# Yujia-Yan/Transkun

Hardware: AMD Instinct MI355X
Metric: semi-CRF logProb+backward steps/sec at T=1024, NBatch=352 (higher is better)
Workload: dtype f32; 1 GPU; NeuralSemiCRFInterval(score, noise).logProb(intervals) fwd+bwd through the public API (Python interval lists packed inside the timed region), T=1024, NBatch=352 per GPU, fp32, exact-hash randn-like scores resident in HBM; T=1024, NBatch=352, impl=0, parallelism=chains sharded, 1 rank(s) seen by the process group, no data-path collective

## Files before the change

include/semicrf_hip.h:

```cpp
#ifndef SEMICRF_HIP_H
#define SEMICRF_HIP_H

#include <stddef.h>
#include <stdint.h>

#ifdef __cplusplus
extern "C" {
#endif

#define SEMICRF_ABI_VERSION 2

#define SEMICRF_OK 0
#define SEMICRF_EINVAL 1
#define SEMICRF_EWORKSPACE 2
#define SEMICRF_ELAUNCH 3
#define SEMICRF_ETIMEOUT 4

#define SEMICRF_OP_LOGZ_FWD 0
#define SEMICRF_OP_LOGZ_BWD 1
#define SEMICRF_OP_VITERBI 2
#define SEMICRF_OP_EVAL_PATH 3
#define SEMICRF_OP_INTERVAL_SCORE 4
#define SEMICRF_OP_SAMPLE 5
#define SEMICRF_OP_VITERBI_NBEST 6
// ... 13 lines not shown

#define SEMICRF_SCORE_BF16X3 4
#define SEMICRF_LEN_BF16X3 16

typedef void* semicrf_stream_t;

int semicrf_abi_version(void);
const char* semicrf_last_error(void);
size_t semicrf_workspace_bytes(int op, int T, int B);

int semicrf_workspace_register(void* ws, size_t ws_bytes);
int semicrf_workspace_unregister(void* ws);

void semicrf_set_impl(int impl);
int semicrf_get_impl(void);

int semicrf_debug_device_status(void);

int semicrf_async_error(void);

int semicrf_debug_wg_ticket(int n_spine, int grid, int block);

void semicrf_debug_score_variant(int variant);

int semicrf_logz_fwd(const float* score, const float* noise, int T, int B,
                     float* logZ, float* v, void* ws, size_t ws_bytes, semicrf_stream_t stream);

int semicrf_logz_bwd(const float* score, const float* noise, const float* v, const float* logZ,
                     const float* gout, int T, int B, float* dScore, float* dNoise, float* q_out,
                     void* ws, size_t ws_bytes, semicrf_stream_t stream);
// ... 261 lines not shown
```

transkun_amd/_lib.py:

```python
from __future__ import annotations

import collections
import ctypes
import os
from typing import Optional

import torch

_HERE = os.path.dirname(os.path.abspath(__file__))
LIB_PATH = os.environ.get("SEMICRF_LIB") or os.path.join(_HERE, "libsemicrf_hip.so")

OP_LOGZ_FWD, OP_LOGZ_BWD, OP_VITERBI, OP_EVAL_PATH, OP_INTERVAL_SCORE, OP_SAMPLE, OP_VITERBI_NBEST, OP_POSTERIORS = range(8)
OP_MARGINAL_DECODE = 8
OP_EXPECTATION = 9
OP_MBR_SELECT = 10
OP_MARGINAL_DECODE_TOL = 11
OP_ATTRIBUTE_HEADS = 12
OP_ATTRIBUTE_HEADS_BWD = 13
HEADS_ROW_TILE = 64
HEADS_SLICE = 64
HEADS_BWD_ROW_CHUNK = 512
ATTENTION_MAX_L = 256
ATTENTION_MAX_D = 64
TOL_MAX = 8
# ... 15 lines not shown
                ("step", ctypes.c_float), ("rectified", ctypes.c_int32), ("pad_", ctypes.c_int32)]


class AdaBeliefGroups(ctypes.Structure):
    _fields_ = [("n", ctypes.c_int32), ("pad_", ctypes.c_int32), ("g", AdaBeliefGroup * OPTIM_MAX_GROUPS)]


_SIGS = {
    "semicrf_abi_version": (ctypes.c_int, []),
    "semicrf_last_error": (ctypes.c_char_p, []),
    "semicrf_workspace_bytes": (_sz, [_i, _i, _i]),
    "semicrf_workspace_register": (_i, [_vp, _sz]),
    "semicrf_workspace_unregister": (_i, [_vp]),
    "semicrf_set_impl": (None, [_i]),
    "semicrf_get_impl": (ctypes.c_int, []),
    "semicrf_debug_device_status": (ctypes.c_int, []),
    "semicrf_async_error": (ctypes.c_int, []),
    "semicrf_logz_bwd_f": (_i, [_vp, _vp, _vp, _vp, _vp, _i, _i, _vp, _vp, _vp, _i, _vp, _sz, _vp]),
    "semicrf_logprob_bwd_f": (_i, [_vp, _vp, _vp, _vp, _vp, _i, _i, _i, _vp, _i64, _vp, _vp, _vp, _i, _vp, _sz, _vp]),
    "semicrf_logprob_path_table_supported": (_i, [_i, _i]),
    "semicrf_logprob_fwd_t": (_i, [_vp, _vp, _i, _i, _vp, _i64, _vp, _vp, _vp, _vp, _vp, _vp, _sz, _vp]),
    "semicrf_logprob_bwd_t": (_i, [_vp, _vp, _vp, _vp, _vp, _i, _i, _i, _vp, _i64, _vp, _vp, _vp, _i, _vp, _vp, _sz, _vp]),
    "semicrf_debug_wg_ticket": (_i, [_i, _i, _i]),
    "semicrf_debug_score_variant": (None, [_i]),
    "semicrf_logz_fwd": (_i, [_vp, _vp, _i, _i, _vp, _vp, _vp, _sz, _vp]),
    "semicrf_logz_bwd": (_i, [_vp, _vp, _vp, _vp, _vp, _i, _i, _vp, _vp, _vp, _vp, _sz, _vp]),
    "semicrf_viterbi": (_i, [_vp, _vp, _i, _i, _vp, _i, _vp, _i64, _vp, _vp, _sz, _vp]),
    "semicrf_sample": (_i, [_vp, _vp, _vp, _i, _i, _i64, _i, ctypes.c_uint64, _vp, _vp, _i64, _vp, _vp, _sz, _vp]),
    "semicrf_viterbi_nbest": (_i, [_vp, _vp, _i, _i, _i, _vp, _i, _vp, _i64, _vp, _vp, _vp, _vp, _sz, _vp]),
    "semicrf_posteriors": (_i, [_vp, _vp, _vp, _vp, _vp, _i, _i, _vp, _vp, _vp, _vp, _vp, _vp, _vp, _sz, _vp]),
# ... 190 lines not shown
    with torch.cuda.device(device):
        rc = load().semicrf_workspace_register(ctypes.c_void_p(ws.data_ptr()), ctypes.c_size_t(ws.numel()))
    if rc != 0:
        check(rc, "semicrf_workspace_register")
    _LEASES[key] = ws
    while len(_LEASES) > _LEASE_MAX:
        _, old = _LEASES.popitem(last=False)
        load().semicrf_workspace_unregister(ctypes.c_void_p(old.data_ptr()))
    return ws


def set_impl(impl: int) -> None:
    load().semicrf_set_impl(int(impl))


def device_status() -> int:
    return int(load().semicrf_debug_device_status())


def async_error() -> int:
    return int(load().semicrf_async_error())


def get_impl() -> int:
    return int(load().semicrf_get_impl())
```

transkun_amd/csrc/api.hip:

```cpp
#include <stdarg.h>
#include <string.h>
#include <stdlib.h>
#include <atomic>
#include <mutex>
#include <unordered_map>
#include "common.h"
#include "attention_math.h"

namespace semicrf {

static thread_local char g_err[512] = "";
static std::atomic<int> g_impl{0};

void set_error(const char* fmt, ...)
{
    va_list ap;
    va_start(ap, fmt);
    vsnprintf(g_err, sizeof(g_err), fmt, ap);
    va_end(ap);
}

void launch_rowseq_sweep(int mode, int dir, const float* score, const float* noise, int T, int B, float* u,
                         int* code, float* out_last, hipStream_t stream);
void launch_marginals(const float* score, const float* noise, const float* v, const float* q,
// ... 81 lines not shown
                   const float* bias, const float* w2, const float* b2, int zero_cols, int accumulate, hipStream_t stream);
size_t proj_tn_workspace_bytes(long long M, int R, int N);
size_t proj_nn3_workspace_bytes(int K, int N);
int launch_proj_nn3(const float* A, long long lda, long long M, int K, const float* B, long long ldb, int N, float* out, long long ldout,
                    const float* bias, const float* w2, const float* b2, int zero_cols, int accumulate, void* ws, size_t ws_bytes,
                    hipStream_t stream);
void launch_merge_weights_fwd(const float* W, const float* bias, int D, int size, int rows, float* Wm, float* bm, float* WmT, hipStream_t stream);
void launch_merge_weights_bwd(const float* W, const float* bias, const float* dWm, const float* dbm, int D, int size, float* dW, float* dbias,
                              float* ws, hipStream_t stream);
size_t merge_weights_bwd_workspace_bytes(int size);
void launch_stage_linear(const float* W, const float* bias, int D, int size, int rows_pad, float* BT, float* Wqd, float* w2, float* b2,
                         hipStream_t stream);
int launch_proj_tn(const float* A, long long lda, long long M, int R, int extra_col0, int total_rows, const float* X, long long ldx, int N,
                   float* dW, long long lddw, float* db, void* ws, size_t ws_bytes, hipStream_t stream);
size_t persist_workspace_bytes(int T, int B);
size_t sample_workspace_bytes(int T, int nB);
size_t posterior_workspace_bytes(int T, int B);
size_t expectation_workspace_bytes(int T, int B);
void launch_alpha_from(const float* score, const float* noise, const int* start, int T, int B, float* v, float* logZ, hipStream_t stream);
void launch_expectation(const float* score, const float* noise, const float* weight, const float* nweight, const float* v, const float* q,
                        int T, int B, float* E, float* H, void* ws, hipStream_t stream);
void launch_covariance(const float* score, const float* noise, const float* weight, const float* nweight, const float* gout, int T, int B,
                       float* C, float* Cn, const void* ws, hipStream_t stream);
void launch_posteriors(const float* score, const float* noise, const float* v, const float* q, const float* logZ, int T, int B,
                       float* node, float* begin, float* end, float* single, float* noiseP, float* entropy, void* ws,
                       hipStream_t stream);
void launch_interval_marginals(const float* score, const float* v, const float* q, const float* logZ, int T, int B, const int* pairs,
                               int K, const int* offsets, float* out, hipStream_t stream);
size_t marginal_decode_workspace_bytes(int T, int B);
void launch_marginal_decode(const float* score, const float* v, const float* q, const float* logZ, int T, int B, const float* tau,
// ... 131 lines not shown
    std::lock_guard<std::mutex> lk(g_lease_mu);
    auto it = g_leases.find(ws);
    if (it != g_leases.end()) it->second.clean = false;
}

}

using namespace semicrf;

extern "C" {

int semicrf_abi_version(void) { return SEMICRF_ABI_VERSION; }
const char* semicrf_last_error(void) { return g_err; }
void semicrf_set_impl(int impl) { g_impl.store(impl); }
int semicrf_get_impl(void) { return g_impl.load(); }
int semicrf_debug_device_status(void) { return read_and_clear_device_status(); }
int semicrf_async_error(void) { return (int)take_async_error(); }
int semicrf_debug_wg_ticket(int n_spine, int grid, int block) { return persist_wg_ticket(n_spine, grid, block); }
void semicrf_debug_score_variant(int variant) { set_score_variant(variant); }

int semicrf_workspace_register(void* ws, size_t ws_bytes)
{
    SEMICRF_CHECK_ARG(ws != nullptr && ws_bytes > 0, "workspace is NULL or empty");
    if (ensure_abort_word(nullptr)) { set_error("could not hand the abort word to the device"); return SEMICRF_ELAUNCH; }
    std::lock_guard<std::mutex> lk(g_lease_mu);
    g_leases[ws] = Lease{ws_bytes, -1, 0, 0, false, 0u};
    return SEMICRF_OK;
}

int semicrf_workspace_unregister(void* ws)
// ... 1124 lines not shown
```

transkun_amd/csrc/persist.hip:

```cpp
#include <atomic>
#include <stdlib.h>
#include "common.h"
#include "pathscore.h"

#ifndef SEMICRF_PANEL_PROBES
#define SEMICRF_PANEL_PROBES 0
#endif

#ifndef SEMICRF_PROBE_TASKS
#define SEMICRF_PROBE_TASKS 0
#endif
#ifndef SEMICRF_PROBE_HIST
#define SEMICRF_PROBE_HIST 0
#endif

#ifndef SEMICRF_CT_DBG
#define SEMICRF_CT_DBG -1
#endif

namespace semicrf {

constexpr int PB = 16;
#ifndef SEMICRF_RING
#define SEMICRF_RING 4
// ... 14 lines not shown
#endif
#ifndef SEMICRF_BANDX_WGSTRIDE
#define SEMICRF_BANDX_WGSTRIDE 3
#endif
#ifndef SEMICRF_BANDX_WAVES
#define SEMICRF_BANDX_WAVES 1
#endif
#ifndef SEMICRF_BANDX_K0
#define SEMICRF_BANDX_K0 8
#endif
constexpr int NBT = RING + NNEAR;
constexpr int FAR0 = RING + NNEAR;
constexpr int RS = 4;
constexpr int GS = RS;
constexpr int GP = 32;
#ifndef SEMICRF_TPT
#define SEMICRF_TPT 12
#endif
constexpr int TPT = SEMICRF_TPT;
#ifndef SEMICRF_LEADT
#define SEMICRF_LEADT 4
#endif
constexpr int LEADT = SEMICRF_LEADT;
__host__ __device__ inline int nfull_of(int q) { return q + 1 - LEADT >= 0 ? (q + 1 - LEADT) / TPT : 0; }
__host__ __device__ inline int nparts_of(int q) { return nfull_of(q) + 1; }
__host__ __device__ inline void part_tiles(int q, int part, int& m0, int& m1)
{
    m0 = part * TPT;
    m1 = part < nfull_of(q) ? m0 + TPT : q + 1;
}
#ifndef SEMICRF_NT
#define SEMICRF_NT 640
#endif
constexpr int NT = SEMICRF_NT;
constexpr int MAX_CHUNKS = 16;
constexpr float LOG2E = 1.4426950408889634f;
constexpr float LN2 = 0.6931471805599453f;
constexpr int SPIN_LIMIT = 1 << 20;
constexpr int SPIN_LIMIT_LDS = 1 << 24;
constexpr float RESC_LIFT = 96.0f, RESC_HI = 108.0f, RESC_EARLY = 56.0f;
constexpr unsigned CTRL_INIT = 0xffffffffu;
constexpr unsigned U_EMPTY = 0xffffffffu;

constexpr size_t CTRL_WORDS = 256;
constexpr int CTRL_EXIT = 64;
// ... 19 lines not shown
    int panelWaves;
    int hybridPanelWaves;
    int hybridStart;
    int zeroWaves;
    unsigned tag;
    int selfclean;
    unsigned expect_gen;
    unsigned dbg;
    unsigned* ctrl;
    u64* ts;
    unsigned* ug;
    unsigned* ug_other;
    int gradLazyShort;
    int bandWaves;
    u64* farg;
    float* u_out;
    float* last_out;
    int* code;
    const float* vfwd;
    const float* logZ;
    const float* gout;
    int gstride;
    float gscale;
    float* dScore;
    float* dNoise;
    const int* pathPairs;
    const int* pathOffsets;
    int pathK;
    int pathSpine;
    float* pathOut;
// ... 18 lines not shown
__device__ __forceinline__ u64 make_granule(unsigned tag, float v)
{
    return ((u64)tag << 32) | (u64)__float_as_uint(v);
}
__device__ __forceinline__ u64 make_granule_key(unsigned tag, float v, int key)
{
    return ((u64)(((tag & 0xffffu) << 16) | ((unsigned)key & 0xffffu)) << 32) | (u64)__float_as_uint(v);
}
__device__ __forceinline__ void store_granule(u64* p, u64 g)
{
    __hip_atomic_store(p, g, __ATOMIC_RELAXED, __HIP_MEMORY_SCOPE_AGENT);
}
__device__ __forceinline__ u64 load_granule(const u64* p)
{
    return __hip_atomic_load(p, __ATOMIC_RELAXED, __HIP_MEMORY_SCOPE_AGENT);
}

template <typename Tp>
__device__ __forceinline__ Tp kernarg_again(size_t off)
{
    typedef __attribute__((address_space(4))) const char ka_t;
    ka_t* ka = (ka_t*)__builtin_amdgcn_kernarg_segment_ptr();
    asm volatile("" : "+s"(ka));
    return *(__attribute__((address_space(4))) const Tp*)(ka + off);
}

template <int DIR>
__device__ __forceinline__ int frame_of(int p, int T) { return DIR == 0 ? p : T - 1 - p; }

template <int DIR>
// ... 340 lines not shown
    int* const fcons = (int*)(lds + LDS_CTL) + NRBUF + RING + NNSLOT + fw;
    float* const dScore = P.dScore;
    float gz = 0.f, lzc = 0.f;
    if (GRAD && NNEAR > 0 && cvalid) { gz = P.gout[(size_t)c * P.gstride] * P.gscale; lzc = P.logZ[c]; }
    __builtin_amdgcn_s_setprio(SEMICRF_FAR_PRIO);
    const bool fprobe = SEMICRF_PANEL_PROBES && (DBGF(P) & 16u) && cbase_is_first && lane == 0;
    const int nfar = NNEAR > 0 ? NFARW : __builtin_amdgcn_readfirstlane(P.nfarw);
    if (fw >= nfar) return;
    for (int k = RING + fw; k < K; k += nfar) {
        if (fprobe && k < 64) P.ts[640 + k] = __builtin_amdgcn_s_memrealtime();
        const int prow = k * PB + r;
        const bool rvalid = cvalid && prow < T;
        const int prow_c = prow < T ? prow : T - 1;
        float aM = SEMICRF_NEG_INF, aS = 0.f;
        int aK = 0x7fffffff;
        const int nparts = k >= FAR0 ? nparts_of(k - FAR0) : 0;
        u64 eq[4] = {0, 0, 0, 0};
        if (SEMICRF_FAR_EARLY && rvalid && nparts > 0) {
#pragma unroll
            for (int i = 0; i < 4; ++i)
                if (i < nparts) eq[i] = load_granule(farg + ((size_t)i * T + prow) * Bs + c);
        }
        float ncell[NNEAR > 0 ? NNEAR : 1][PB];
        float arow = 0.f;
        if (NNEAR > 0) {
            int spins = 0;
            while (lds_flag_load(nready + k % NNSLOT) != k + 1) {
                __builtin_amdgcn_s_sleep(1);
                if (spin_abort(ctrl, spins, SPIN_LIMIT_LDS, 11)) break;
            }
            const char* nb = lds + LDS_NEAR + (k % NNSLOT) * NEAR_SLOT_BYTES;
#pragma unroll
            for (int n = 0; n < NNEAR; ++n)
#pragma unroll
                for (int u = 0; u < PB; ++u) ncell[n][u] = *(const float*)(nb + n * TILE_BYTES + u * (PB * RS * 4) + (r * RS + ch) * 4);
            if (GRAD) arow = rvalid ? (((const float*)(nb + NNEAR * TILE_BYTES))[lane] - lzc) * LOG2E : 0.f;
// ... 50 lines not shown
                }
            }
        }
        if (fprobe && k < 64) P.ts[832 + k] = __builtin_amdgcn_s_memrealtime();
        if (rvalid && nparts > 0) {
            for (int p0 = 0; p0 < nparts; p0 += 4) {
                const int np = nparts - p0 < 4 ? nparts - p0 : 4;
                u64 gq[4];
                bool have[4] = {false, false, false, false};
                int spins = 0;
                bool first = SEMICRF_FAR_EARLY && p0 == 0;
                while (true) {
#pragma unroll
                    for (int i = 0; i < 4; ++i)
                        if (i < np && !have[i])
                            gq[i] = first ? eq[i] : load_granule(farg + ((size_t)(p0 + i) * T + prow) * Bs + c);
                    first = false;
                    bool all = true;
#pragma unroll
                    for (int i = 0; i < 4; ++i)
                        if (i < np && !have[i]) {
                            const bool ok = MODE == 0 ? (unsigned)(gq[i] >> 32) == tag : (unsigned)(gq[i] >> 48) == (tag & 0xffffu);
                            if (ok) have[i] = true;
                            else all = false;
                        }
                    if (all) break;
                    __builtin_amdgcn_s_sleep(1);
                    if (spin_abort(ctrl, spins, SPIN_LIMIT, 3)) break;
                }
#pragma unroll
                for (int i = 0; i < 4; ++i)
// ... 311 lines not shown
                    gr = load_granule(pathg + c);
                    if ((unsigned)(gr >> 32) == ptag) break;
                    __builtin_amdgcn_s_sleep(8);
                    if (spin_abort(ctrl, spins, SPIN_LIMIT, 15)) { ok = false; break; }
                }
                pathOut[c] = ok ? __uint_as_float((unsigned)gr) - mine * sc : __uint_as_float(0x7fc00000u);
            }
            if (GRAD) {
                float dv = gz * fexp2(arow + mine + draw - 2.0f * sp);
                if (pdiag) dv = dv + nadd;
                dScore[((size_t)frow * T + frow) * Bs + c] = dv;
            }
            if (MODE == 1) code[(size_t)c * T + frow] = (mykey + 1) | (sp > 0.0f ? 0x40000000 : 0);
        }
        if (SEMICRF_PANEL_PROBES && trace) ts[k] = __builtin_amdgcn_s_memrealtime();
    }
}

#ifndef SEMICRF_GRAD_AUX
#define SEMICRF_GRAD_AUX 2
#endif
constexpr int GRAD_AUX = SEMICRF_GRAD_AUX;
#ifndef SEMICRF_CELL_AUX
#define SEMICRF_CELL_AUX 2
#endif
constexpr int CELL_AUX = SEMICRF_CELL_AUX;
#ifndef SEMICRF_PNS
#define SEMICRF_PNS 3
#endif
constexpr int PNS = SEMICRF_PNS;
// ... 89 lines not shown
                 : "v"(addr), "n"(0 * XR + 0 * XH), "n"(0 * XR + 1 * XH), "n"(1 * XR + 0 * XH), "n"(1 * XR + 1 * XH),
                   "n"(2 * XR + 0 * XH), "n"(2 * XR + 1 * XH), "n"(3 * XR + 0 * XH), "n"(3 * XR + 1 * XH));
}
__device__ __forceinline__ void panel_wait_younger(int y)
{
    if (y >= 44) wait_vmcnt<44>();
    else if (y >= 36) wait_vmcnt<36>();
    else if (y >= 28) wait_vmcnt<28>();
    else if (y >= 20) wait_vmcnt<20>();
    else if (y >= 10) wait_vmcnt<10>();
    else wait_vmcnt<0>();
}

struct PanelTask { int k, part, g, q4; };

__device__ __forceinline__ void panel_tt_decode(int tt, PanelTask& t)
{
    if (tt < LEADT - 1) { t.part = 0; t.k = FAR0 + tt; return; }
    tt -= LEADT - 1;
    int a = 0;
    while (tt >= TPT * (a + 1) * (a + 2) / 2) ++a;
    tt -= TPT * a * (a + 1) / 2;
    const int q = a * TPT + tt / (a + 1) + LEADT - 1;
    t.part = tt % (a + 1);
    t.k = FAR0 + q;
}
__device__ __forceinline__ void panel_task_decode(const SweepParams& P, int task, PanelTask& t)
{
    t.q4 = task & 3;
    const int t2 = task >> 2;
    t.g = t2 % P.nPanelGroups;
    panel_tt_decode(t2 / P.nPanelGroups, t);
}

__device__ __forceinline__ bool panel_next_task(const SweepParams& P, PanelTask& t)
{
    int task = 0;
    if ((threadIdx.x & 63) == 0) task = (int)(atomicAdd(P.ctrl + 2, 1u) + 1u);
    task = __builtin_amdgcn_readfirstlane(task) + P.taskBase;
    if (task >= P.nTasks) return false;
    panel_task_decode(P, task, t);
    return true;
}

template <int MODE, int DIR, bool GRAD>
__device__ __forceinline__ void panel_role(const SweepParams& P, char* lds, int wslot, int hist_role = 0, int first_task = -1)
{
// ... 34 lines not shown
    while (true) {
        PanelTask tk;
        if (first_task >= 0 && first_task < P.nTasks) {
            panel_task_decode(P, first_task, tk);
#if SEMICRF_STAGGER > 0
            for (int i = 0, n = tk.k - FAR0 < 48 ? tk.k - FAR0 : 48; i < n; ++i) __builtin_amdgcn_s_sleep(SEMICRF_STAGGER);
#endif
        } else if (!panel_next_task(P, tk)) break;
        first_task = -1;
        if (SEMICRF_PROBE_TASKS && (dbg & 256u) && tk.k == RING && tk.part == 0 && tk.g == 0 && tk.q4 == 0) tracer = true;
        u64* const tsp = P.ts + (3 * T) / 2 + 5 * tn;
        const bool tr = SEMICRF_PROBE_TASKS && tracer && lane == 0 && 5 * tn + 5 <= T / 2;
        if (tr) tsp[0] = __builtin_amdgcn_s_memrealtime();
        const int q = tk.k - FAR0;
        int m0, m1;
        part_tiles(q, tk.part, m0, m1);
        const int k = tk.k, part = tk.part, g = tk.g, q4 = tk.q4;
        const int pbase = k * PB + q4 * 4;
        if (pbase >= T) continue;
        const int c = c0 + g * GP + q8 * 4;
        const bool cvalid = c < c1;
        const int cl = cvalid ? c : c0;

        float aM[4][4], aS[4][4];
        int aK[4][4];
#pragma unroll
        for (int rr = 0; rr < 4; ++rr)
#pragma unroll
            for (int i = 0; i < 4; ++i) { aM[rr][i] = SEMICRF_NEG_INF; aS[rr][i] = 0.f; aK[rr][i] = 0x7fffffff; }

        float arow[4][4], gz[4];
// ... 216 lines not shown
            if (tprobe) { P.ts[1664 + k] = __builtin_amdgcn_s_memrealtime(); P.ts[1792 + k] = (u64)npoll; }
            if (refill) {
                panel_fetch_cells<DIR>(score, G, stage, m + PNS, T, Bs, cell_nt);
                if (!probe_stream && !probe_nou) panel_fetch_gran<false>(ursrc, stage, G.gvoff, m + PNS, B);
                issued += 10;
                if (s == 0) mark0 = issued; else if (s == 1) mark1 = issued; else mark2 = issued;
            }
        }
        if (tr) { tsp[2] = __builtin_amdgcn_s_memrealtime(); tsp[4] = (u64)(m1 - m0) | ((u64)k << 8) | ((u64)(frontier ? 1 : 0) << 16) | ((u64)part << 20); }
        if (!(GRAD && MODE == 0)) wait_vmcnt<0>();
        (void)frontier;
        if (SEMICRF_PANEL_PROBES && (dbg & 16u) && g == 0 && q4 == 0 && m1 == q + 1 && lane == 0 && k < 64 && T >= 1024)
            P.ts[1728 + k] = __builtin_amdgcn_s_memrealtime();

        const bool b5 = (lane & 32) != 0, b4 = (lane & 16) != 0, b3 = (lane & 8) != 0;
        u64* fbase = farg + (size_t)part * T * Bs;
        const int pi = pbase + (b5 ? 2 : 0) + (b4 ? 1 : 0);
        {
            constexpr int RSTR = 65 * 8;
            char* const rb = stage0;
#pragma unroll
            for (int rr = 0; rr < 4; ++rr)
#pragma unroll
                for (int i = 0; i < 4; ++i)
                    *(float2*)(rb + (rr * 4 + i) * RSTR + lane * 8) =
                        make_float2(aM[rr][i], MODE == 0 ? aS[rr][i] : __int_as_float(aK[rr][i]));
            const int orow = (b5 ? 2 : 0) + (b4 ? 1 : 0);
#pragma unroll
            for (int e = 0; e < 2; ++e) {
                const int oi = (b3 ? 2 : 0) + e;
                const char* src = rb + (orow * 4 + oi) * RSTR + q8 * 8;
// ... 18 lines not shown
                    gr = make_granule_key(tag, bm, bk);
                }
                if (pi < T && cc < c1 && !(SEMICRF_PANEL_PROBES && (dbg & 32u))) store_granule(fbase + (size_t)pi * Bs + cc, gr);
            }
        }
        if (SEMICRF_PANEL_PROBES && (dbg & 16u) && g == 0 && m1 == q + 1 && lane == 0 && k < 64)
            P.ts[256 + 64 * q4 + k] = __builtin_amdgcn_s_memrealtime();
        if (PFOLD && pathfix) {
            asm volatile("s_waitcnt vmcnt(0)" ::: "memory");
            const int* const ptab2 = kernarg_again<const int*>(offsetof(SweepParams, ptab));
            const float* const gout2 = kernarg_again<const float*>(offsetof(SweepParams, gout));
            float* const dScore2 = kernarg_again<float*>(offsetof(SweepParams, dScore));
            const int gstride2 = kernarg_again<int>(offsetof(SweepParams, gstride));
            const float wpath = kernarg_again<float>(offsetof(SweepParams, noiseAdd));
            int f0, f1;
            part_tiles(k - FAR0, part, f0, f1);
#pragma nounroll
            for (int n = 0; n < 16; ++n) {
                const int prow = pbase + (n >> 2), ci = c + (n & 3);
                if (prow >= T) break;
                const int fb = frame_of<DIR>(prow, T);
                const int pend = ptab2[(size_t)fb * Bs + (ci < c1 ? ci : c1 - 1)] & PTAB_NONE;
                const int pj = T - 1 - pend;
                if (ci < c1 && (unsigned)(pj - f0 * PB) < (unsigned)((f1 - f0) * PB) && (pj & 7) == (lane >> 3)) {
                    float* const cell = dScore2 + ((size_t)pend * T + fb) * Bs + ci;
                    const float mv = __hip_atomic_load(cell, __ATOMIC_RELAXED, __HIP_MEMORY_SCOPE_AGENT);
                    const float nv = mv + wpath * gout2[(size_t)ci * gstride2];
                    if (grad_nt) __builtin_nontemporal_store(nv, cell);
                    else *cell = nv;
                }
            }
        }
        if (tr) tsp[3] = __builtin_amdgcn_s_memrealtime();
        ++tn;
    }
}

__device__ __forceinline__ void zero_row(float* __restrict__ dScore, int e, int T, int B, int lane)
{
    const size_t n = (size_t)(T - 1 - e) * B;
    float* rowp = dScore + ((size_t)e * T + e + 1) * B;
    const size_t lead = (4 - (((uintptr_t)rowp >> 2) & 3)) & 3;
    const size_t head = lead < n ? lead : n;
    const size_t n4 = (n - head) / 4;
    typedef float f32x4 __attribute__((ext_vector_type(4)));
    f32x4* v = (f32x4*)(rowp + head);
    const f32x4 z = {0.f, 0.f, 0.f, 0.f};
    for (size_t i = lane; i < n4; i += 64) __builtin_nontemporal_store(z, v + i);
    if ((size_t)lane < head) rowp[lane] = 0.f;
    const size_t tail0 = head + n4 * 4;
// ... 365 lines not shown
#ifndef SEMICRF_NFARW2_MINT
#define SEMICRF_NFARW2_MINT 1024
#endif
#ifndef SEMICRF_NT_MISALIGNED
#define SEMICRF_NT_MISALIGNED 0
#endif
static bool cell_policy_nt(int T, int nb, int min_mb)
{
    const double mb = 4.0 * nb * ((double)T * (T + 1) / 2) / 1e6;
    return mb >= (double)min_mb;
}

static int max_parts(int T)
{
    const int K = (T + PB - 1) / PB;
    return K > FAR0 ? nparts_of(K - 1 - FAR0) : 1;
}

__global__ __launch_bounds__(256) void zero_upper_kernel(float* __restrict__ dScore, int T, int B)
{
    const int e = blockIdx.y;
    const size_t n = (size_t)(T - 1 - e) * B;
    float* rowp = dScore + ((size_t)e * T + e + 1) * B;
    const size_t lead = (4 - (((uintptr_t)rowp >> 2) & 3)) & 3;
    const size_t head = lead < n ? lead : n;
    const size_t n4 = (n - head) / 4;
    float4* v = (float4*)(rowp + head);
    for (size_t i = (size_t)blockIdx.x * 256 + threadIdx.x; i < n4; i += (size_t)gridDim.x * 256)
        v[i] = make_float4(0.f, 0.f, 0.f, 0.f);
    if (blockIdx.x == 0) {
        if (threadIdx.x < head) rowp[threadIdx.x] = 0.f;
// ... 28 lines not shown
{
    static std::atomic<int> ncu[MAX_DEVICES];
    const int dev = current_device();
    int n = ncu[dev].load();
    if (n == 0) {
        int v = 0;
        n = 256;
        if (hipDeviceGetAttribute(&v, hipDeviceAttributeMultiprocessorCount, dev) == hipSuccess && v > 0) n = v;
        ncu[dev].store(n);
    }
    return n;
}

size_t persist_workspace_bytes(int T, int B)
{
    return CTRL_BYTES + align_up((size_t)2 * T * sizeof(u64)) + (size_t)max_parts(T) * align_up((size_t)T * B * sizeof(u64)) +
           2 * align_up((size_t)T * B * sizeof(unsigned)) +
           align_up((size_t)B * sizeof(u64)) +
           band_flag_bytes(T, B) + band_copy_bytes(T, B);
}

bool persist_supported(int T, int B)
{
    return B >= 2 && T >= 2 && T < 65535 && (long long)T * B * 64 < (1ll << 31) &&
           (B + GS - 1) / GS <= MAX_CHUNKS * (device_cus() / 2 > 0 ? device_cus() / 2 : 1);
}

static unsigned next_tag()
{
    static std::atomic<unsigned> counter{0};
    const unsigned lo = (counter.fetch_add(1) % 65534u) + 1u;
// ... 47 lines not shown
        P.gstride = grad->gstride; P.gscale = grad->gscale; P.noiseAdd = grad->noise_add;
    }
    P.score = score; P.noise = noise; P.T = T; P.B = B; P.K = (T + PB - 1) / PB;
    P.band = nullptr; P.bandFlags = nullptr; P.bandSpines = (B + GS - 1) / GS; P.bandGroups = (B + GP - 1) / GP; P.bandK0 = 0; P.copyWaves = 0;
    P.tag = lease_tag ? (lease_tag % 65534u) + 1u : next_tag();
    P.dbg = 0u;
    P.selfclean = 0;
#if SEMICRF_PANEL_PROBES
    if (const char* dbg = getenv("SEMICRF_DEBUG_FLAGS")) P.dbg = (unsigned)atoi(dbg);
    if (SEMICRF_CT_DBG >= 0) P.dbg = (unsigned)SEMICRF_CT_DBG;
#endif
    char* w = (char*)ws;
    P.ts = (u64*)(w + CTRL_BYTES);
    const size_t ts_bytes = align_up((size_t)2 * T * sizeof(u64));
    P.farg = (u64*)(w + CTRL_BYTES + ts_bytes);
    const size_t ug_off = CTRL_BYTES + ts_bytes + (size_t)max_parts(T) * align_up((size_t)T * B * sizeof(u64));
    const size_t ug_bytes = align_up((size_t)T * B * sizeof(unsigned));
    const unsigned upar = lease != 0 ? (lease_tag & 1u) : 0u;
    P.ug = (unsigned*)(w + ug_off + upar * ug_bytes);
    P.ug_other = nullptr;
    const size_t band_off = ug_off + 2 * ug_bytes + align_up((size_t)B * sizeof(u64));
    const bool band_ok = band_in_sweep(T, B);
    if (path && mode == 0 && dir == 0 && !grad) {
        P.pathPairs = path->pairs ? path->pairs : path->offsets; P.pathOffsets = path->offsets; P.pathK = path->K; P.pathOut = path->out;
        P.ptabOut = path->ptab;
        P.pathg = (u64*)(w + ug_off + 2 * ug_bytes);
    }
    P.u_out = u_out; P.last_out = last_out; P.code = code;
    const size_t fill_bytes = (SEMICRF_PANEL_PROBES && (P.dbg & 512u)) ? ug_off : persist_workspace_bytes(T, B) - band_copy_bytes(T, B);
    if (P.dbg != 0u) lease = lease ? 1 : 0;
    if (lease != 2) hipLaunchKernelGGL(fill_ff_kernel, dim3(1024), dim3(256), 0, stream, (v4u*)ws, (fill_bytes + 15) / 16);
// ... 5 lines not shown
    const int ncu = device_cus();
    const int nSpineTotal = (B + GS - 1) / GS;
    const int maxSpine = ncu / 2 > 0 ? ncu / 2 : 1;
    const int nchunks = (nSpineTotal + maxSpine - 1) / maxSpine;
    if (nchunks > MAX_CHUNKS) return 1;
    int perChunk = (nSpineTotal + nchunks - 1) / nchunks;
    perChunk = (perChunk + GP / GS - 1) / (GP / GS) * (GP / GS);
    if (perChunk > maxSpine) perChunk = maxSpine / (GP / GS) * (GP / GS) > 0 ? maxSpine / (GP / GS) * (GP / GS) : maxSpine;
    for (int ci = 0; ci < nchunks; ++ci) {
        P.c0 = ci * perChunk * GS;
        P.c1 = P.c0 + perChunk * GS < B ? P.c0 + perChunk * GS : B;
        if (P.c0 >= P.c1) break;
        const int nb = P.c1 - P.c0;
        P.nSpine = (nb + GS - 1) / GS;
        P.nPanelGroups = (nb + GP - 1) / GP;
        long long ntask = 0;
        for (int q = 0; q < P.K - FAR0; ++q) ntask += nparts_of(q);
        ntask *= 4;
        P.nTasks = (int)(ntask * P.nPanelGroups);
        P.ctrl = (unsigned*)w + (size_t)ci * CTRL_WORDS;
        const int nSpineWG = (P.nSpine + SPH - 1) / SPH;
        int nPanelWG = ncu - nSpineWG;
        if (nPanelWG < 0) nPanelWG = 0;
        int hpw = HPW_MAX > 0 ? HPW_MAX : 0;
        if (knobs.hybrid_waves >= 0 && knobs.hybrid_waves <= HPW_MAX) hpw = knobs.hybrid_waves;
        int hstart = grad ? SEMICRF_GRAD_HSTART : P.K * 5 / 8;
        hstart = hstart < 8 ? 8 : (hstart > 40 ? 40 : hstart);
        if (knobs.hybrid_start >= 0) hstart = knobs.hybrid_start;
        P.hybridStart = hstart;
        P.hybridPanelWaves = hpw;
        int pw = (T >= 1024 && nb >= 256) ? PW_MAX : (PW_MAX < 4 ? PW_MAX : 4);
        if (knobs.panel_waves > 0) pw = knobs.panel_waves;
        if (pw < 1) pw = 1;
        if (pw > PW_MAX) pw = PW_MAX;
// ... 22 lines not shown
        P.nfarw = (!grad && nb <= SEMICRF_NFARW2_MAXB && T >= SEMICRF_NFARW2_MINT && NFARW >= 2) ? 2 : 1;
        if (knobs.nfarw >= 1 && knobs.nfarw <= NFARW) P.nfarw = knobs.nfarw;
        P.cellNT = cell_policy_nt(T, B, SEMICRF_NT_MIN_MB) ? 1 : 0;
        if (!SEMICRF_NT_MISALIGNED && grad && B % 32 != 0) P.cellNT = 0;
        P.gradNT = cell_policy_nt(T, B, SEMICRF_GRAD_NT_MIN_MB) ? 1 : 0;
        if (P.nTasks == 0) nPanelWG = 0;
        P.pathSpine = nPanelWG == 0 ? 1 : 0;
        P.band = nullptr; P.copyWaves = 0;
        if (band_ok && !grad && nchunks == 1 && nPanelWG > 0 && NT / 64 - pw - zw - bw - 1 >= SEMICRF_BANDX_WAVES) {
            P.bandFlags = (unsigned*)(w + band_off);
            P.band = (float*)(w + band_off + band_flag_bytes(T, B));
            P.bandK0 = SEMICRF_BANDX_K0;
            P.copyWaves = SEMICRF_BANDX_WAVES;
        }
        const int grid = nSpineWG + nPanelWG;
        P.taskBase = nPanelWG * P.panelWaves;
        if (P.taskBase > P.nTasks) P.taskBase = P.nTasks;
        if (grad) launch_one<0, 1, true>(P, grid, stream);
        else if (mode == 0 && dir == 0) launch_one<0, 0, false>(P, grid, stream);
        else if (mode == 0 && dir == 1) launch_one<0, 1, false>(P, grid, stream);
        else if (mode == 1 && dir == 0) launch_one<1, 0, false>(P, grid, stream);
        else launch_one<1, 1, false>(P, grid, stream);
    }
    return 0;
}

int launch_persist_sweep(int mode, int dir, const float* score, const float* noise, int T, int B, float* u_out,
                         float* last_out, int* code, void* ws, hipStream_t stream, int lease, unsigned lease_tag)
{
    return launch_persist_sweep_impl(mode, dir, score, noise, T, B, u_out, last_out, code, ws, stream, nullptr, lease, lease_tag);
// ... 56 lines not shown
```

Before: 1877 steps/s.

## Split tail panel tasks into finer parts for better end-of-sweep load balance

Adds an end-geometry scheme so the last few panel columns of the persistent sweep use a smaller tiles-per-task value. Their far partials land in a separate workspace region, which raises task count and shortens the serial tail at the end of the sweep. The task decoding, partial-buffer addressing and workspace sizing are generalised to handle both geometries, and a host knob plus a query for the chosen geometry are exposed. In exchange it adds more partial granules to reduce, extra per-task decode work, and a larger workspace.

```diff
diff --git a/include/semicrf_hip.h b/include/semicrf_hip.h
--- a/include/semicrf_hip.h
+++ b/include/semicrf_hip.h
@@ -51,6 +51,9 @@
 
 void semicrf_set_impl(int impl);
 int semicrf_get_impl(void);
+
+void semicrf_set_end_tasks(int end_k, int end_tpt);
+void semicrf_last_end_tasks(int* q0, int* tpt);
 
 int semicrf_debug_device_status(void);
 
diff --git a/transkun_amd/_lib.py b/transkun_amd/_lib.py
--- a/transkun_amd/_lib.py
+++ b/transkun_amd/_lib.py
@@ -53,6 +53,8 @@
     "semicrf_workspace_unregister": (_i, [_vp]),
     "semicrf_set_impl": (None, [_i]),
     "semicrf_get_impl": (ctypes.c_int, []),
+    "semicrf_set_end_tasks": (None, [_i, _i]),
+    "semicrf_last_end_tasks": (None, [ctypes.POINTER(ctypes.c_int), ctypes.POINTER(ctypes.c_int)]),
     "semicrf_debug_device_status": (ctypes.c_int, []),
     "semicrf_async_error": (ctypes.c_int, []),
     "semicrf_logz_bwd_f": (_i, [_vp, _vp, _vp, _vp, _vp, _i, _i, _vp, _vp, _vp, _i, _vp, _sz, _vp]),
@@ -273,6 +275,16 @@
     load().semicrf_set_impl(int(impl))
 
 
+def set_end_tasks(end_k: int = -1, end_tpt: int = -1) -> None:
+    load().semicrf_set_end_tasks(int(end_k), int(end_tpt))
+
+
+def last_end_tasks():
+    q0, tpt = ctypes.c_int(-1), ctypes.c_int(0)
+    load().semicrf_last_end_tasks(ctypes.byref(q0), ctypes.byref(tpt))
+    return q0.value, tpt.value
+
+
 def device_status() -> int:
     return int(load().semicrf_debug_device_status())
 
diff --git a/transkun_amd/csrc/api.hip b/transkun_amd/csrc/api.hip
--- a/transkun_amd/csrc/api.hip
+++ b/transkun_amd/csrc/api.hip
@@ -119,6 +119,8 @@
 int launch_proj_tn(const float* A, long long lda, long long M, int R, int extra_col0, int total_rows, const float* X, long long ldx, int N,
                    float* dW, long long lddw, float* db, void* ws, size_t ws_bytes, hipStream_t stream);
 size_t persist_workspace_bytes(int T, int B);
+void persist_set_end_tasks(int endK, int endTPT);
+void persist_last_end_tasks(int* q0, int* tpt);
 size_t sample_workspace_bytes(int T, int nB);
 size_t posterior_workspace_bytes(int T, int B);
 size_t expectation_workspace_bytes(int T, int B);
@@ -280,6 +282,8 @@
 const char* semicrf_last_error(void) { return g_err; }
 void semicrf_set_impl(int impl) { g_impl.store(impl); }
 int semicrf_get_impl(void) { return g_impl.load(); }
+void semicrf_set_end_tasks(int end_k, int end_tpt) { persist_set_end_tasks(end_k, end_tpt); }
+void semicrf_last_end_tasks(int* q0, int* tpt) { persist_last_end_tasks(q0, tpt); }
 int semicrf_debug_device_status(void) { return read_and_clear_device_status(); }
 int semicrf_async_error(void) { return (int)take_async_error(); }
 int semicrf_debug_wg_ticket(int n_spine, int grid, int block) { return persist_wg_ticket(n_spine, grid, block); }
diff --git a/transkun_amd/csrc/persist.hip b/transkun_amd/csrc/persist.hip
--- a/transkun_amd/csrc/persist.hip
+++ b/transkun_amd/csrc/persist.hip
@@ -2,6 +2,7 @@
 #include <stdlib.h>
 #include "common.h"
 #include "pathscore.h"
+#include "sweep_geom.h"
 
 #ifndef SEMICRF_PANEL_PROBES
 #define SEMICRF_PANEL_PROBES 0
@@ -52,21 +53,6 @@
 constexpr int RS = 4;
 constexpr int GS = RS;
 constexpr int GP = 32;
-#ifndef SEMICRF_TPT
-#define SEMICRF_TPT 12
-#endif
-constexpr int TPT = SEMICRF_TPT;
-#ifndef SEMICRF_LEADT
-#define SEMICRF_LEADT 4
-#endif
-constexpr int LEADT = SEMICRF_LEADT;
-__host__ __device__ inline int nfull_of(int q) { return q + 1 - LEADT >= 0 ? (q + 1 - LEADT) / TPT : 0; }
-__host__ __device__ inline int nparts_of(int q) { return nfull_of(q) + 1; }
-__host__ __device__ inline void part_tiles(int q, int part, int& m0, int& m1)
-{
-    m0 = part * TPT;
-    m1 = part < nfull_of(q) ? m0 + TPT : q + 1;
-}
 #ifndef SEMICRF_NT
 #define SEMICRF_NT 640
 #endif
@@ -116,6 +102,9 @@
     int gradLazyShort;
     int bandWaves;
     u64* farg;
+    EndGeom endg;
+    u64* fargEnd;
+    int endRows, endRow0;
     float* u_out;
     float* last_out;
     int* code;
@@ -164,6 +153,15 @@
 __device__ __forceinline__ u64 load_granule(const u64* p)
 {
     return __hip_atomic_load(p, __ATOMIC_RELAXED, __HIP_MEMORY_SCOPE_AGENT);
+}
+
+constexpr int CTRL_STAMPQ = 224;
+__device__ __forceinline__ void drain_stamp(const SweepParams& P, unsigned kind)
+{
+    const u64 now = __builtin_amdgcn_s_memrealtime();
+    const unsigned slot = atomicAdd(P.ctrl + CTRL_STAMPQ, 1u) + 1u;
+    if (slot < 2u * (unsigned)P.T)
+        P.ts[slot] = (now & 0x00ffffffffffffffull) | ((u64)(__builtin_amdgcn_s_getreg(6164) & 7) << 56) | ((u64)kind << 60);
 }
 
 template <typename Tp>
@@ -534,12 +532,15 @@
         const int prow_c = prow < T ? prow : T - 1;
         float aM = SEMICRF_NEG_INF, aS = 0.f;
         int aK = 0x7fffffff;
-        const int nparts = k >= FAR0 ? nparts_of(k - FAR0) : 0;
+        const int nparts = k >= FAR0 ? nparts_of(k - FAR0, P.endg) : 0;
+        const bool kend = k - FAR0 >= P.endg.q0;
+        const u64* const farg0 = kend ? P.fargEnd + (size_t)(prow - P.endRow0) * Bs + c : farg + (size_t)prow * Bs + c;
+        const size_t fstride = (size_t)(kend ? P.endRows : T) * Bs;
         u64 eq[4] = {0, 0, 0, 0};
         if (SEMICRF_FAR_EARLY && rvalid && nparts > 0) {
 #pragma unroll
             for (int i = 0; i < 4; ++i)
-                if (i < nparts) eq[i] = load_granule(farg + ((size_t)i * T + prow) * Bs + c);
+                if (i < nparts) eq[i] = load_granule(farg0 + (size_t)i * fstride);
         }
         float ncell[NNEAR > 0 ? NNEAR : 1][PB];
         float arow = 0.f;
@@ -620,7 +621,7 @@
 #pragma unroll
                     for (int i = 0; i < 4; ++i)
                         if (i < np && !have[i])
-                            gq[i] = first ? eq[i] : load_granule(farg + ((size_t)(p0 + i) * T + prow) * Bs + c);
+                            gq[i] = first ? eq[i] : load_granule(farg0 + (size_t)(p0 + i) * fstride);
                     first = false;
                     bool all = true;
 #pragma unroll
@@ -962,6 +963,7 @@
             if (MODE == 1) code[(size_t)c * T + frow] = (mykey + 1) | (sp > 0.0f ? 0x40000000 : 0);
         }
         if (SEMICRF_PANEL_PROBES && trace) ts[k] = __builtin_amdgcn_s_memrealtime();
+        if (SEMICRF_PANEL_PROBES && (dbg & 2048u) && k == K - 1 && lane == 0) drain_stamp(P, 1u);
     }
 }
 
@@ -1081,23 +1083,11 @@
 
 struct PanelTask { int k, part, g, q4; };
 
-__device__ __forceinline__ void panel_tt_decode(int tt, PanelTask& t)
-{
-    if (tt < LEADT - 1) { t.part = 0; t.k = FAR0 + tt; return; }
-    tt -= LEADT - 1;
-    int a = 0;
-    while (tt >= TPT * (a + 1) * (a + 2) / 2) ++a;
-    tt -= TPT * a * (a + 1) / 2;
-    const int q = a * TPT + tt / (a + 1) + LEADT - 1;
-    t.part = tt % (a + 1);
+__device__ __forceinline__ void panel_task_decode(const SweepParams& P, int task, PanelTask& t)
+{
+    int q;
+    panel_task_split(task, P.nPanelGroups, P.endg, q, t.part, t.g, t.q4);
     t.k = FAR0 + q;
-}
-__device__ __forceinline__ void panel_task_decode(const SweepParams& P, int task, PanelTask& t)
-{
-    t.q4 = task & 3;
-    const int t2 = task >> 2;
-    t.g = t2 % P.nPanelGroups;
-    panel_tt_decode(t2 / P.nPanelGroups, t);
 }
 
 __device__ __forceinline__ bool panel_next_task(const SweepParams& P, PanelTask& t)
@@ -1162,7 +1152,7 @@
         if (tr) tsp[0] = __builtin_amdgcn_s_memrealtime();
         const int q = tk.k - FAR0;
         int m0, m1;
-        part_tiles(q, tk.part, m0, m1);
+        part_tiles(q, tk.part, P.endg, m0, m1);
         const int k = tk.k, part = tk.part, g = tk.g, q4 = tk.q4;
         const int pbase = k * PB + q4 * 4;
         if (pbase >= T) continue;
@@ -1409,7 +1399,12 @@
             P.ts[1728 + k] = __builtin_amdgcn_s_memrealtime();
 
         const bool b5 = (lane & 32) != 0, b4 = (lane & 16) != 0, b3 = (lane & 8) != 0;
-        u64* fbase = farg + (size_t)part * T * Bs;
+        const EndGeom eg{kernarg_again<int>(offsetof(SweepParams, endg) + offsetof(EndGeom, q0)),
+                         kernarg_again<int>(offsetof(SweepParams, endg) + offsetof(EndGeom, tpt)), 0};
+        u64* fbase = k - FAR0 >= eg.q0
+                         ? kernarg_again<u64*>(offsetof(SweepParams, fargEnd)) +
+                               ((long long)part * kernarg_again<int>(offsetof(SweepParams, endRows)) - kernarg_again<int>(offsetof(SweepParams, endRow0))) * (long long)Bs
+                         : farg + (size_t)part * T * Bs;
         const int pi = pbase + (b5 ? 2 : 0) + (b4 ? 1 : 0);
         {
             constexpr int RSTR = 65 * 8;
@@ -1458,7 +1453,7 @@
             const int gstride2 = kernarg_again<int>(offsetof(SweepParams, gstride));
             const float wpath = kernarg_again<float>(offsetof(SweepParams, noiseAdd));
             int f0, f1;
-            part_tiles(k - FAR0, part, f0, f1);
+            part_tiles(k - FAR0, part, eg, f0, f1);
 #pragma nounroll
             for (int n = 0; n < 16; ++n) {
                 const int prow = pbase + (n >> 2), ci = c + (n & 3);
@@ -1478,6 +1473,7 @@
         if (tr) tsp[3] = __builtin_amdgcn_s_memrealtime();
         ++tn;
     }
+    if (SEMICRF_PANEL_PROBES && (dbg & 2048u) && lane == 0) drain_stamp(P, 0u);
 }
 
 __device__ __forceinline__ void zero_row(float* __restrict__ dScore, int e, int T, int B, int lane)
@@ -1873,7 +1869,30 @@
 static int max_parts(int T)
 {
     const int K = (T + PB - 1) / PB;
-    return K > FAR0 ? nparts_of(K - 1 - FAR0) : 1;
+    return K > FAR0 ? nparts_of(K - 1 - FAR0, EndGeom{END_OFF, TPT, 0}) : 1;
+}
+static size_t end_part_bytes(int T, int B)
+{
+    const int K = (T + PB - 1) / PB;
+    return align_up((size_t)end_rows_capacity(K - FAR0) * B * sizeof(u64));
+}
+static size_t far_partial_bytes(int T, int B)
+{
+    const int K = (T + PB - 1) / PB;
+    return (size_t)max_parts(T) * align_up((size_t)T * B * sizeof(u64)) + (size_t)end_parts_capacity(K - FAR0) * end_part_bytes(T, B);
+}
+
+static std::atomic<int> g_end_k{-1}, g_end_tpt{-1};
+static std::atomic<int> g_last_end_q0{-1}, g_last_end_tpt{0};
+void persist_set_end_tasks(int endK, int endTPT)
+{
+    g_end_k.store(endK);
+    g_end_tpt.store(endTPT);
+}
+void persist_last_end_tasks(int* q0, int* tpt)
+{
+    *q0 = g_last_end_q0.load();
+    *tpt = g_last_end_tpt.load();
 }
 
 __global__ __launch_bounds__(256) void zero_upper_kernel(float* __restrict__ dScore, int T, int B)
@@ -1932,7 +1951,7 @@
 
 size_t persist_workspace_bytes(int T, int B)
 {
-    return CTRL_BYTES + align_up((size_t)2 * T * sizeof(u64)) + (size_t)max_parts(T) * align_up((size_t)T * B * sizeof(u64)) +
+    return CTRL_BYTES + align_up((size_t)2 * T * sizeof(u64)) + far_partial_bytes(T, B) +
            2 * align_up((size_t)T * B * sizeof(unsigned)) +
            align_up((size_t)B * sizeof(u64)) +
            band_flag_bytes(T, B) + band_copy_bytes(T, B);
@@ -2010,7 +2029,9 @@
     P.ts = (u64*)(w + CTRL_BYTES);
     const size_t ts_bytes = align_up((size_t)2 * T * sizeof(u64));
     P.farg = (u64*)(w + CTRL_BYTES + ts_bytes);
-    const size_t ug_off = CTRL_BYTES + ts_bytes + (size_t)max_parts(T) * align_up((size_t)T * B * sizeof(u64));
+    P.fargEnd = (u64*)(w + CTRL_BYTES + ts_bytes + (size_t)max_parts(T) * align_up((size_t)T * B * sizeof(u64)));
+    P.endRows = end_rows_capacity(P.K - FAR0);
+    const size_t ug_off = CTRL_BYTES + ts_bytes + far_partial_bytes(T, B);
     const size_t ug_bytes = align_up((size_t)T * B * sizeof(unsigned));
     const unsigned upar = lease != 0 ? (lease_tag & 1u) : 0u;
     P.ug = (unsigned*)(w + ug_off + upar * ug_bytes);
@@ -2046,10 +2067,9 @@
         const int nb = P.c1 - P.c0;
         P.nSpine = (nb + GS - 1) / GS;
         P.nPanelGroups = (nb + GP - 1) / GP;
-        long long ntask = 0;
-        for (int q = 0; q < P.K - FAR0; ++q) ntask += nparts_of(q);
-        ntask *= 4;
-        P.nTasks = (int)(ntask * P.nPanelGroups);
+        P.endg = EndGeom{END_OFF, TPT, 0x7fffffff};
+        P.endRow0 = 0;
+        P.nTasks = (int)(4 * panel_tt_count(P.K - FAR0, P.endg) * P.nPanelGroups);
         P.ctrl = (unsigned*)w + (size_t)ci * CTRL_WORDS;
         const int nSpineWG = (P.nSpine + SPH - 1) / SPH;
         int nPanelWG = ncu - nSpineWG;
@@ -2102,6 +2122,16 @@
             P.copyWaves = SEMICRF_BANDX_WAVES;
         }
         const int grid = nSpineWG + nPanelWG;
+        if (nPanelWG > 0) {
+            const int nq = P.K - FAR0, ek = g_end_k.load(), et = g_end_tpt.load();
+            P.endg = ek < 0 ? end_geometry(nq, P.nPanelGroups, nPanelWG * pw + nSpineWG * hpw) : end_geometry_of(nq, ek, et);
+            if (P.endg.q0 != END_OFF) {
+                P.endRow0 = (FAR0 + P.endg.q0) * PB;
+                P.nTasks = (int)(4 * panel_tt_count(nq, P.endg) * P.nPanelGroups);
+            }
+        }
+        g_last_end_q0.store(P.endg.q0 != END_OFF ? P.endg.q0 : -1);
+        g_last_end_tpt.store(P.endg.q0 != END_OFF ? P.endg.tpt : 0);
         P.taskBase = nPanelWG * P.panelWaves;
         if (P.taskBase > P.nTasks) P.taskBase = P.nTasks;
         if (grad) launch_one<0, 1, true>(P, grid, stream);
diff --git a/transkun_amd/csrc/sweep_geom.h b/transkun_amd/csrc/sweep_geom.h
--- /dev/null
+++ b/transkun_amd/csrc/sweep_geom.h
@@ -0,0 +1,118 @@
+#pragma once
+
+#ifndef SEMICRF_HD
+#if defined(__HIPCC__) || defined(__CUDACC__)
+#define SEMICRF_HD __host__ __device__
+#else
+#define SEMICRF_HD
+#endif
+#endif
+
+namespace semicrf {
+
+#ifndef SEMICRF_TPT
+#define SEMICRF_TPT 12
+#endif
+constexpr int TPT = SEMICRF_TPT;
+#ifndef SEMICRF_LEADT
+#define SEMICRF_LEADT 4
+#endif
+constexpr int LEADT = SEMICRF_LEADT;
+
+constexpr int END_OFF = 0x7fffffff;
+struct EndGeom {
+    int q0;
+    int tpt;
+    int tt0;
+};
+
+SEMICRF_HD inline int nfull_of(int q, const EndGeom& e)
+{
+    if (q + 1 - LEADT < 0) return 0;
+    return q >= e.q0 ? (q + 1 - LEADT) / e.tpt : (q + 1 - LEADT) / TPT;
+}
+SEMICRF_HD inline int nparts_of(int q, const EndGeom& e) { return nfull_of(q, e) + 1; }
+SEMICRF_HD inline void part_tiles(int q, int part, const EndGeom& e, int& m0, int& m1)
+{
+    const int tpt = q >= e.q0 ? e.tpt : TPT;
+    m0 = part * tpt;
+    m1 = part < nfull_of(q, e) ? m0 + tpt : q + 1;
+}
+
+SEMICRF_HD inline void panel_tt_decode(int tt, const EndGeom& e, int& q, int& part)
+{
+    if (tt >= e.tt0) {
+        tt -= e.tt0;
+        int qq = e.q0;
+        for (int n = nparts_of(qq, e); tt >= n; n = nparts_of(qq, e)) { tt -= n; ++qq; }
+        q = qq; part = tt;
+        return;
+    }
+    if (tt < LEADT - 1) { part = 0; q = tt; return; }
+    tt -= LEADT - 1;
+    int a = 0;
+    while (tt >= TPT * (a + 1) * (a + 2) / 2) ++a;
+    tt -= TPT * a * (a + 1) / 2;
+    q = a * TPT + tt / (a + 1) + LEADT - 1;
+    part = tt % (a + 1);
+}
+
+SEMICRF_HD inline void panel_task_split(int task, int groups, const EndGeom& e, int& q, int& part, int& g, int& q4)
+{
+    q4 = task & 3;
+    const int t2 = task >> 2;
+    g = t2 % groups;
+    panel_tt_decode(t2 / groups, e, q, part);
+}
+
+inline long long panel_tt_count(int nq, const EndGeom& e)
+{
+    long long n = 0;
+    for (int q = 0; q < nq; ++q) n += nparts_of(q, e);
+    return n;
+}
+
+constexpr int END_K_MAX = 8;
+constexpr int END_TPT_MIN = 4;
+constexpr int END_PARTS_MAX = 8;
+constexpr int END_MIN_NQ = 16;
+constexpr int END_TASKS_PER_WAVE = 4;
+
+inline int end_rows_capacity(int nq) { return nq >= 1 ? (nq < END_K_MAX ? nq : END_K_MAX) * 16 : 0; }
+inline int end_parts_capacity(int nq)
+{
+    if (nq < 1) return 0;
+    const int bulk_parts = nq >= LEADT ? (nq - LEADT) / TPT + 1 : 1;
+    const int fit = bulk_parts * (nq + 3) * 16 / end_rows_capacity(nq);
+    return fit < 1 ? 1 : (fit > END_PARTS_MAX ? END_PARTS_MAX : fit);
+}
+
+inline EndGeom end_geometry_of(int nq, int endK, int endTPT)
+{
+    EndGeom off{END_OFF, TPT, 0x7fffffff};
+    if (endK <= 0 || endTPT < 1 || endTPT >= TPT || nq < 1) return off;
+    if (endK > END_K_MAX) endK = END_K_MAX;
+    if (endK > nq) endK = nq;
+    EndGeom e{nq - endK, endTPT, 0};
+    if (nparts_of(nq - 1, e) > end_parts_capacity(nq)) return off;
+    e.tt0 = (int)panel_tt_count(e.q0, off);
+    return e;
+}
+
+constexpr int END_TPT = 2 * TPT / 3;
+constexpr int END_EXTRA_PARTS = 6;
+inline EndGeom end_geometry(int nq, int groups, int waves)
+{
+    const EndGeom off{END_OFF, TPT, 0x7fffffff};
+    if (nq < END_MIN_NQ || groups < 1 || waves < 1 || END_TPT < END_TPT_MIN) return off;
+    if (4 * groups * panel_tt_count(nq, off) < (long long)END_TASKS_PER_WAVE * waves) return off;
+    const int extra = (nq - LEADT) / END_TPT - (nq - LEADT) / TPT;
+    if (extra < 1) return off;
+    int k = END_EXTRA_PARTS / extra;
+    if (k < 2) k = 2;
+    if (k > END_K_MAX) k = END_K_MAX;
+    return end_geometry_of(nq, k, END_TPT);
+}
+
+
+}
```

New measurement: 1873 steps/s. No clear change (-0.2%).
